# chensh236/ComputerVisionImageStich2

Measured on AMD Instinct MI355X. Metric: warp+blend MPix/s at 4096x4096x3 f32, higher is better.
Workload: dtype f32 (f64 accumulators)

## Files before the change

computervisionimagestich2_amd/capi.py:

```python
import ctypes as C
import os
import re

import numpy as np

_HERE = os.path.dirname(os.path.abspath(__file__))
LIB_PATH = os.environ.get("STITCH_LIB", os.path.join(_HERE, "libstitch_hip.so"))

KERNELS = ("compose", "seam", "mask", "vv_x_fwd", "vv_x_bwd", "vv_y_fwd", "vv_y_bwd", "decimate", "collapse_top", "collapse",
           "collapse_l0", "vv_xbyf", "vv_x_fwd_src", "coarse")
KERNEL_SYMBOLS = {"compose": "k_src_index (source-fused) / k_compose", "seam": "k_seam", "mask": "k_mask", "vv_x_fwd": "k_vv_x_fwd<T, false, false>", "vv_x_bwd": "k_vv_x_bwd",
                  "vv_y_fwd": "k_vv_y_fwd1 / k_vv_y_fwd", "vv_y_bwd": "k_vv_y_bwd_dec", "decimate": "k_decimate", "collapse_top": "k_blend_top",
                  "collapse": "k_collapse<float, false>", "collapse_l0": "k_collapse<T, true>", "vv_xbyf": "k_vv_xbyf<false, float, 0, false>", "vv_x_fwd_src": "k_vv_x_fwd<T, true, false>",
                  "coarse": "k_coarse"}


class StitchError(RuntimeError):
    def __init__(self, code, text):
        super().__init__(f"stitch error {code}: {text}")
        self.code = code


OK, ERR_ARG, ERR_EMPTY_MIDROW, ERR_ZERO_OVERLAP, ERR_PYRAMID, ERR_HIP, ERR_NO_DEVICE = 0, -1, -2, -3, -4, -5, -6
ERR_NO_MAP, ERR_CAPACITY = -7, -8
# ... 101 lines not shown
)

RIG_EXPOSURE_SIGNATURES = _signatures(
    ("stitch_rig_create_exposure", i32, vp, i32, i32, vp, i32, vp, vp, vp), ("stitch_rig_from_panorama_exposure", i32, vp, vp, i32, vp, vp, vp),
    ("stitch_dev_rig_stitch_exposure_u8", i32, vp, vp, i32, vp, vp, vp, vp, vp),
    ("stitch_dev_transfer_many_u8", i32, vp, vp, vp, i32, i32, i32, i32, i32, i32, i32, vp, vp, vp),
)

CALIBRATE_SIGNATURES = _signatures(
    ("stitch_calibrate_opts_default stitch_calibration_destroy", None, vp), ("stitch_dev_calibrate_u8", i32, vp, i32, i32, vp, vp, vp),
    ("stitch_dev_calibrate_from_features_u8", i32, vp, vp, i32, i32, vp, vp, vp), ("stitch_calibrate_u8", i32, vp, i32, i32, vp, vp),
    ("stitch_calibration_info", i32, vp, vp, vp, vp, vp, vp, vp), ("stitch_calibration_step_at", i32, vp, i32, vp),
    ("stitch_calibration_counts", i32, vp, vp, vp), ("stitch_calibration_step_support", i32, vp, i32, vp, vp),
    ("stitch_rig_from_calibration", i32, vp, vp, vp, vp),
)

RIG_SEAMS_SIGNATURES = _signatures(
    ("stitch_seam_from_sums", i32, i32, i32, i32, i32, i32, i32, vp), ("stitch_dev_pairs_seamed_*", i32, vp, vp, i32, vp, vp),
    ("stitch_rig_fix_seams stitch_rig_seams", i32, vp, vp, i32), ("stitch_rig_clear_seams", i32, vp),
    ("stitch_dev_rig_geometric_seams", i32, vp, vp, vp), ("stitch_dev_rig_coverage_u8", i32, vp, i32, i32, vp, vp),
    ("stitch_rig_step_canvas", i32, vp, i32, vp, vp),
)

_lib = None


def lib():
    global _lib
    if _lib is None:
        if not os.path.exists(LIB_PATH):
            raise ImportError(f"{LIB_PATH} is missing: build it with `python -c 'import __graft_entry__ as g; g.build()'` "
                              "(make -C computervisionimagestich2_amd/csrc). There is no CPU fallback.")
        try:
            import torch
        except ImportError:
            pass
        L = C.CDLL(LIB_PATH)
        for name, (res, args) in list(SIGNATURES.items()) + list(PANORAMA_SIGNATURES.items()) + list(RIG_SIGNATURES.items()) + list(EXPOSURE_SIGNATURES.items()) \
                + list(RIG_EXPOSURE_SIGNATURES.items()) + list(CALIBRATE_SIGNATURES.items()) + list(RIG_SEAMS_SIGNATURES.items()):
            try:
                f = getattr(L, name)
            except AttributeError:
                raise ImportError(f"{LIB_PATH} does not export {name}: it was built from another include/stitch.h") from None
            f.restype, f.argtypes = res, args
        L.stitch_plan_handoff_counts.restype, L.stitch_plan_handoff_counts.argtypes = i32, [vp, vp]
        if hasattr(L, "stitch_plan_g_flag_counts"):
            L.stitch_plan_g_flag_counts.restype, L.stitch_plan_g_flag_counts.argtypes = i32, [vp, vp]
        if hasattr(L, "stitch_plan_mask_row_counts"):
            L.stitch_plan_mask_row_counts.restype, L.stitch_plan_mask_row_counts.argtypes = i32, [vp, vp]
        if hasattr(L, "stitch_plan_index_counts"):
            L.stitch_plan_index_counts.restype, L.stitch_plan_index_counts.argtypes = i32, [vp, vp]
        _lib = L
    return _lib


def _chk(rc):
    if rc < 0:
        raise StitchError(rc, lib().stitch_last_error().decode())
    return rc


def _p(a):
    return a.ctypes.data_as(C.c_void_p)


def _fn(stem, a):
    sfx = {"uint8": "u8", "float32": "f32"}.get(str(a.dtype).rpartition(".")[2])
    if sfx is None:
        raise TypeError(f"unsupported pixel type {a.dtype}")
    return getattr(lib(), stem + sfx)


def _img(a):
    a = np.ascontiguousarray(a)
# ... 730 lines not shown
    _chk(lib().stitch_dev_finish_u8(_dp(result), result.shape[2], result.shape[1], num, den, _dp(hist), _stream()))
    return result


def dev_synth(w, h, frame_id, dtype, device=None):
    import torch
    out = torch.empty((3, h, w), dtype=dtype, device=device or torch.device("cuda", torch.cuda.current_device()))
    _chk(_fn("stitch_dev_synth_", out)(_dp(out), int(w), int(h), int(frame_id), _stream()))
    return out


def dev_check_fastdiv(w):
    t, m = C.c_ulonglong(), C.c_ulonglong()
    _chk(lib().stitch_dev_check_fastdiv(w, C.byref(t), C.byref(m)))
    return t.value, m.value


def dev_check_collapse_taps(w, h, probe):
    t, m = C.c_ulonglong(), C.c_ulonglong()
    _chk(lib().stitch_dev_check_collapse_taps(int(w), int(h), int(probe), C.byref(t), C.byref(m)))
    return t.value, m.value


def dev_quantize(src, out=None):
    import torch
    assert src.is_cuda and src.is_contiguous() and src.dtype == torch.float32
    out = torch.empty(src.shape, dtype=torch.uint8, device=src.device) if out is None else out
    _chk(lib().stitch_dev_quantize_u8(_dp(src), _dp(out), src.numel(), _stream()))
    return out


class _Handle:

    def close(self):
        if self._h:
            getattr(lib(), self._destroy)(self._h)
            self._h = C.c_void_p()

    def __del__(self):
        try:
            self.close()
        except Exception:
            pass


class Plan(_Handle):
# ... 96 lines not shown
    def clear_fault(self):
        _chk(lib().stitch_plan_clear_fault(self._h))

    def handoff_counts(self):
        out = (C.c_uint64 * 3)()
        _chk(lib().stitch_plan_handoff_counts(self._h, out))
        return tuple(int(v) for v in out)

    def g_flag_counts(self):
        out = (C.c_uint64 * 2)()
        _chk(lib().stitch_plan_g_flag_counts(self._h, out))
        return tuple(int(v) for v in out)

    def mask_row_counts(self):
        out = (C.c_uint64 * 2)()
        _chk(lib().stitch_plan_mask_row_counts(self._h, out))
        return tuple(int(v) for v in out)

    def index_counts(self):
        out = (C.c_uint32 * 3)()
        _chk(lib().stitch_plan_index_counts(self._h, out))
        return tuple(int(v) for v in out)

    def set_handoff_spin_limit(self, polls):
        _chk(lib().stitch_plan_set_handoff_spin_limit(self._h, int(polls)))

    def set_profiling_kernel(self, name):
        _chk(lib().stitch_plan_set_profiling_kernel(self._h, KERNELS.index(name)))

    def set_profiling(self, on):
        _chk(lib().stitch_plan_set_profiling(self._h, int(bool(on))))

    def read_profile(self):
        ms, n, l0 = (C.c_double * len(KERNELS))(), (C.c_int * len(KERNELS))(), (C.c_double * len(KERNELS))()
        _chk(lib().stitch_plan_read_profile(self._h, ms, n, l0))
        return {KERNELS[i]: (ms[i], n[i], l0[i]) for i in range(len(KERNELS))}


class Band(_Handle):
    _destroy = "stitch_band_destroy"

    def __init__(self, cw, ch, rank, nranks, split_levels, opts=None):
        self._h = C.c_void_p()
        _chk(lib().stitch_band_create(int(cw), int(ch), int(rank), int(nranks), int(split_levels), C.byref(_opts(opts)), C.byref(self._h)))
        self.cw, self.ch, self.rank, self.nranks, self.split_levels = int(cw), int(ch), int(rank), int(nranks), int(split_levels)
        tot = C.c_int()
# ... 346 lines not shown
```

computervisionimagestich2_amd/csrc/k_pyramid.inc:

```
__global__ __launch_bounds__(64) void k_deriche(float* __restrict__ data, float* __restrict__ Y, int N, size_t off,
                                                size_t line_stride, long lines_per_plane, size_t ps, long lines, DRK k) {
    const long line = (long)blockIdx.x * WAVE + threadIdx.x;
    if (line >= lines) return;
    const long plane = line / lines_per_plane, li = line % lines_per_plane;
    float* ptrX = data + plane * ps + li * line_stride;
    float* ptrY = Y + plane * ps + li * line_stride;
    float xp = *ptrX, yb, yp;
    yb = yp = (float)(k.coefp * xp);
    for (int m = 0; m < N; ++m) {
        const float xc = ptrX[(size_t)m * off];
        const float yc = k.a0 * xc + k.a1 * xp - k.b1 * yp - k.b2 * yb;
        ptrY[(size_t)m * off] = yc;
        xp = xc;
        yb = yp;
        yp = yc;
    }
    float xn, xa, yn, ya;
    xn = xa = ptrX[(size_t)(N - 1) * off];
    yn = ya = k.coefn * xn;
    for (int n = N - 1; n >= 0; --n) {
        const float xc = ptrX[(size_t)n * off];
        const float yc = k.a2 * xn + k.a3 * xa - k.b1 * yn - k.b2 * ya;
        xa = xn;
        xn = xc;
// ... 336 lines not shown
    template <typename PX>
    __device__ __forceinline__ NoShift4(const PX*, int, int, int, int, int, int) {}
    __device__ __forceinline__ void issue(int, float[4]) const {}
};
template <typename PX, bool ON>
struct Shift4If {
    typedef NoShift4 type;
};
template <typename PX>
struct Shift4If<PX, true> {
    typedef Shift4<PX> type;
};
template <typename PX, bool AD>
struct SrcRow4 {
    __amdgpu_buffer_rsrc_t fr;
    Shift4<PX> mo;
    typename Shift4If<PX, AD>::type fa;
    __device__ __forceinline__ SrcRow4(const PairArgs<PX>& pa, int pr, int c, int x0, int w)
        : mo(pa.mosaic[pr] + c * ((size_t)pa.mw[pr] * pa.mh[pr]), pa.mw[pr], pa.mh[pr], pa.ox[pr], pa.oy[pr], x0, w),
          fa(pa.frame[pr] + c * ((size_t)pa.fw[pr] * pa.fh[pr]), pa.fw[pr], pa.fh[pr], 0, 0, x0, w) {
        const size_t fe = (size_t)pa.fw[pr] * pa.fh[pr];
        fr = plane_rsrc(pa.frame[pr] + c * fe, fe);
    }
    __device__ __forceinline__ void issue(const u4 idx, int y, float a[4], float b[4]) const {
        if constexpr (AD)
            fa.issue(y, a);
        else {
#pragma unroll
            for (int j = 0; j < 4; ++j) a[j] = buf_raw<PX>(fr, idx[j]);
        }
#if STITCH_C4_ABLATE == 3 || STITCH_C4_ABLATE >= 8
        for (int j = 0; j < 4; ++j) b[j] = (float)y;
#else
        mo.issue(y, b);
#endif
    }
    __device__ __forceinline__ void finish(float a[4], float b[4]) const {
#pragma unroll
        for (int j = 0; j < 4; ++j) {
            a[j] = AD ? raw_to_px<PX>(a[j]) : warped_px<PX>(raw_to_px<PX>(a[j]));
            b[j] = raw_to_px<PX>(b[j]);
        }
    }
};
struct NoSrcRow4 {
    __device__ __forceinline__ NoSrcRow4(const NoPairArgs&, int, int, int, int) {}
    __device__ __forceinline__ void issue(const u4, int, float[4], float[4]) const {}
    __device__ __forceinline__ void finish(float[4], float[4]) const {}
};
template <typename OUT, bool DENSE, bool AD>
struct SrcRow4Of {
    typedef NoSrcRow4 type;
};
template <typename OUT, bool AD>
struct SrcRow4Of<OUT, true, AD> {
    typedef SrcRow4<OUT, AD> type;
};

#ifndef STITCH_C4_WAVES
#define STITCH_C4_WAVES 7
#endif
#ifndef STITCH_C4_PREFETCH
#define STITCH_C4_PREFETCH 0
#endif
#ifndef STITCH_C4_ABLATE
#define STITCH_C4_ABLATE 0
#endif
#ifndef STITCH_C4_OPAQUE_ALPHA
#define STITCH_C4_OPAQUE_ALPHA 1
#endif
typedef __attribute__((address_space(3))) f4 lds_f4;
template <typename OUT, bool DENSE, bool AD, bool GEN, bool MR = false>
__device__ __forceinline__ void collapse_cols4(const CollapseArgs<OUT, DENSE>& A, int c, int x0, int y0, int y1, int pr, float* sh, MaskRowsArg mr = MaskRowsArg{}) {
    const int pitch = A.pitch, sh_ = A.sh, spitch = A.spitch, opitch = A.opitch;
    const size_t ps = A.ps, sps = A.sps, ops = A.ops;
    const ExpandTab& tb = A.tb;
    const SeamDev* __restrict__ seam_l0 = A.seam_l0;
    const float* g = A.g_all + (size_t)collapse_slot(A, pr) * 7 * ps;
    const bool share = !DENSE && !seam_l0 && A.lockstep == 2;
    const float* sa = A.gn_all + ((size_t)pr * 7 + c) * sps;
    const float* sb = sa + 3 * sps;
    const float* se = A.en_all + ((size_t)pr * 3 + c) * sps;
    OUT* __restrict__ out = (DENSE ? A.outs.p[pr] : A.outs.p[0] + (size_t)pr * 3 * ops) + c * ops;
    uint8_t* __restrict__ out8 = DENSE && A.outs.q[pr] ? A.outs.q[pr] + c * ops : nullptr;
    const bool use_src = DENSE && A.use_src;
    const int s0 = tb.ix[x0];
    int o1 = 1, o2 = 1, o3 = 2;
    bool e1 = false, e2 = false, e3 = false;
    if constexpr (GEN) {
        const int4 ix4 = *reinterpret_cast<const int4*>(tb.ix + x0);
        o1 = ix4.y - ix4.x, o2 = ix4.z - ix4.x, o3 = ix4.w - ix4.x;
#ifndef STITCH_C4_NO_ENDTAP
        e1 = ix4.y >= A.sw - 1, e2 = ix4.z >= A.sw - 1, e3 = ix4.w >= A.sw - 1;
#endif
    }
#if STITCH_G_IGNORE_COARSER & 1
    const bool za = false, zb = false;
#else
    const bool za = g_span_flag(A.gzn, A.gncn, pr * 7 + c, s0, s0 + 3), zb = g_span_flag(A.gzn, A.gncn, pr * 7 + 3 + c, s0, s0 + 3);
#endif
#if STITCH_G_IGNORE_OWN & 1
    const bool zga = false, zgb = false;
#else
    const bool zga = !DENSE && g_span_flag(A.gz, A.gnc, pr * 7 + c, x0, x0), zgb = !DENSE && g_span_flag(A.gz, A.gnc, pr * 7 + 3 + c, x0, x0);
#endif
    const unsigned zsa = (unsigned)((size_t)A.zon - ((size_t)pr * 7 + c) * sps), zsb = (unsigned)((size_t)A.zon - ((size_t)pr * 7 + 3 + c) * sps);
    const size_t zg = (size_t)A.zo - (size_t)pr * 7 * ps;
    double axs[4];
    {
        const double2 a01 = *reinterpret_cast<const double2*>(tb.ax + x0), a23 = *reinterpret_cast<const double2*>(tb.ax + x0 + 2);
        axs[0] = a01.x, axs[1] = a01.y, axs[2] = a23.x, axs[3] = a23.y;
    }
    auto xrow = [&](int row, float X[3][4]) {
        const unsigned o = (unsigned)row * (unsigned)spitch + (unsigned)s0;
#if STITCH_C4_ABLATE == 1 || STITCH_C4_ABLATE >= 8
        const f4 v[3] = {f4{0.f, 0.f, 0.f, (float)o}, f4{0.f, 0.f, 0.f, 1.f}, f4{0.f, 0.f, 0.f, 2.f}};
#else
        const f4 v[3] = {*reinterpret_cast<const f4u*>(sa + (za ? zsa : o)), *reinterpret_cast<const f4u*>(sb + (zb ? zsb : o)), *reinterpret_cast<const f4u*>(se + o)};
#endif
#if STITCH_C4_OPAQUE_ALPHA
#pragma unroll
        for (int j = 0; j < 4; ++j) asm volatile("" : "+v"(axs[j]));
#endif
#pragma unroll
        for (int q = 0; q < 3; ++q) {
            if constexpr (GEN) {
                const float x_ = v[q].x, y_ = v[q].y, z_ = v[q].z, w_ = v[q].w;
                X[q][0] = lerp_ref(axs[0], x_, y_);
                const float a1 = o1 ? y_ : x_, a2 = o2 == 0 ? x_ : o2 == 1 ? y_ : z_, a3 = o3 == 0 ? x_ : o3 == 1 ? y_ : z_;
                X[q][1] = lerp_ref(axs[1], a1, e1 ? a1 : o1 ? z_ : y_);
                X[q][2] = lerp_ref(axs[2], a2, e2 ? a2 : o2 == 0 ? y_ : o2 == 1 ? z_ : w_);
                X[q][3] = lerp_ref(axs[3], a3, e3 ? a3 : o3 == 0 ? y_ : o3 == 1 ? z_ : w_);
            } else {
                X[q][0] = lerp_ref(axs[0], v[q].x, v[q].y);
                X[q][1] = lerp_ref(axs[1], v[q].y, v[q].z);
                X[q][2] = lerp_ref(axs[2], v[q].y, v[q].z);
                X[q][3] = lerp_ref(axs[3], v[q].z, v[q].w);
            }
        }
    };
    float X1[3][4], X2[3][4];
    int cur1 = -1, cur2 = -1;
    float m4[4] = {0.f, 0.f, 0.f, 0.f};
    if (seam_l0) {
        const SeamDev sd = seam_l0[pr];
#pragma unroll
        for (int j = 0; j < 4; ++j) m4[j] = mask_step(sd, x0 + j);
    }
    const typename SrcRow4Of<OUT, DENSE, AD>::type src(A.pa, pr, c, x0, A.w);
    bool mrow = false;
    auto row_issue = [&](int y, float ga[4], float gb[4], f4& vm) {
        const unsigned o = (unsigned)y * (unsigned)pitch + (unsigned)x0;
        if constexpr (MR)
            if (y == y0 || (y & 63) == 0) mrow = collapse_mask_row(mr, pr, x0, y);
        const unsigned om = MR && mrow ? (unsigned)x0 : o;
        if (use_src)
#if STITCH_C4_ABLATE == 2
            src.issue(u4{0u, 4u, 8u, 12u}, y, ga, gb);
#elif STITCH_C4_ABLATE >= 6
        {
            const unsigned e = ((unsigned)y * 4096u + (unsigned)(x0 - 2048)) * 4u;
            const u4 calc = x0 >= 2048 ? u4{e, e + 4u, e + 8u, e + 12u} : u4{0xfffffff0u, 0xfffffff0u, 0xfffffff0u, 0xfffffff0u};
            src.issue(c == 0 && STITCH_C4_ABLATE == 6 ? *reinterpret_cast<const u4*>(g + o) : STITCH_C4_ABLATE >= 8 ? u4{0u, 4u, 8u, 12u} : calc, y, ga, gb);
        }
#else
            src.issue(AD ? u4{0u, 0u, 0u, 0u} : *reinterpret_cast<const u4*>(g + o), y, ga, gb);
#endif
        else {
            const f4 va = *reinterpret_cast<const f4*>(g + (zga ? zg : o + c * ps)), vb = *reinterpret_cast<const f4*>(g + (zgb ? zg : o + (3 + c) * ps));
#pragma unroll
            for (int j = 0; j < 4; ++j) ga[j] = va[j], gb[j] = vb[j];
        }
        if (share) {
            if (c == 0) vm = *reinterpret_cast<const f4*>(g + om + 6 * ps);
        } else
#if STITCH_C4_ABLATE == 11
        if (!seam_l0) vm = c == 0 ? *reinterpret_cast<const f4*>(g + o + 6 * ps) : f4{0.5f, 0.5f, 0.5f, 0.5f};
#elif STITCH_C4_ABLATE == 12
        if (!seam_l0) vm = f4{0.5f, 0.5f, 0.5f, (float)y};
#else
        if (!seam_l0) vm = *reinterpret_cast<const f4*>(g + om + 6 * ps);
#endif
    };
    float ga[4], gb[4];
    f4 vm = {0.f, 0.f, 0.f, 0.f};
#if STITCH_C4_PREFETCH
    float gan[4], gbn[4];
    f4 vmn = {0.f, 0.f, 0.f, 0.f};
    row_issue(y0, gan, gbn, vmn);
#endif
    for (int y = y0; y < y1; ++y) {
        if (A.lockstep == 1) __builtin_amdgcn_s_barrier();
        const int iy = tb.iy[y], iy2 = iy < sh_ - 1 ? iy + 1 : iy;
        const double ay = tb.ay[y];
        if (iy != cur1) {
            if (iy == cur2) {
#pragma unroll
                for (int q = 0; q < 3; ++q)
#pragma unroll
                    for (int j = 0; j < 4; ++j) X1[q][j] = X2[q][j];
            } else
                xrow(iy, X1);
            cur1 = iy;
        }
        if (iy2 != cur2) {
            if (iy2 == cur1) {
#pragma unroll
                for (int q = 0; q < 3; ++q)
#pragma unroll
                    for (int j = 0; j < 4; ++j) X2[q][j] = X1[q][j];
            } else
                xrow(iy2, X2);
            cur2 = iy2;
        }
#if STITCH_C4_PREFETCH
#pragma unroll
        for (int j = 0; j < 4; ++j) ga[j] = gan[j], gb[j] = gbn[j];
        vm = vmn;
        if (y + 1 < y1) row_issue(y + 1, gan, gbn, vmn);
#else
        row_issue(y, ga, gb, vm);
#endif
        if (share) {
            lds_f4* slot = (lds_f4*)sh + (y & 1) * WAVE + (threadIdx.x & 63);
            if (c == 0) *slot = vm;
            asm volatile("s_waitcnt lgkmcnt(0)\n\ts_barrier" ::: "memory");
            vm = *slot;
        }
        if (use_src) src.finish(ga, gb);
        if (!seam_l0) {
#pragma unroll
            for (int j = 0; j < 4; ++j) m4[j] = vm[j];
        }
        float v4[4];
#pragma unroll
        for (int j = 0; j < 4; ++j) {
            const float ea = lerp_ref(ay, X1[0][j], X2[0][j]);
            const float eb = lerp_ref(ay, X1[1][j], X2[1][j]);
            const float ee = lerp_ref(ay, X1[2][j], X2[2][j]);
            const float la = ga[j] - ea;
            const float lb = gb[j] - eb;
            const float s_ = blend_ref(la, lb, m4[j]);
            float v = s_ + ee;
            if (v > 255.f)
                v = 255.f;
            else if (v < 0.f)
                v = 0.f;
            v4[j] = v;
        }
#if STITCH_C4_ABLATE == 4
        if (!(v4[0] != v4[0] || v4[3] != v4[3])) continue;
#endif
        if constexpr (DENSE)
        {
#if STITCH_C4_ABLATE == 5
            *reinterpret_cast<f4u*>(&out[(size_t)y * opitch + x0]) = f4u{v4[0], v4[1], v4[2], v4[3]};
            continue;
#endif
            store4<OUT>(&out[(size_t)y * opitch + x0], v4, A.u8_words != 0);
            if (sizeof(OUT) == 4 && out8) store4<uint8_t>(&out8[(size_t)y * opitch + x0], v4, A.u8_words != 0);
        }
        else
            *reinterpret_cast<f4*>(&out[(size_t)y * opitch + x0]) = f4{v4[0], v4[1], v4[2], v4[3]};
    }
}

constexpr int C4_SUB = 8, C4_THREADS = 3 * WAVE;
__host__ __device__ inline int c4_padded_blocks(int nb4, int swizzle) { return swizzle && nb4 >= 8 ? (nb4 + 7) & ~7 : nb4; }
template <typename OUT, bool DENSE, bool AD = false, bool GEN = false, bool MR = false>
__global__ __launch_bounds__(C4_THREADS, STITCH_C4_WAVES) void k_collapse4(CollapseArgs<OUT, DENSE> A, int nb4, int ncb, MaskRowsArg mr = MaskRowsArg{}) {
    const int pr = blockIdx.z;
    __shared__ __attribute__((aligned(16))) float c4_sh[2 * WAVE * 4];
    const int nb4p = c4_padded_blocks(nb4, A.swizzle);
    if ((int)blockIdx.x < nb4p) {
        const int c = __builtin_amdgcn_readfirstlane(threadIdx.x >> 6);
        int blk = blockIdx.x, strip = blockIdx.y;
        const int nb8 = nb4p & ~7;
        const int S8 = (int)gridDim.y & ~7;
        if (A.swizzle >= 2 && blk < nb8 && (int)blockIdx.y < S8) {
            const unsigned first = gridDim.x * (blockIdx.y + gridDim.y * blockIdx.z);
            const int xcd = (int)((first + (unsigned)blk) & 7u), t = (int)blockIdx.y * (nb8 >> 3) + (blk >> 3);
            strip = xcd * (S8 >> 3) + t / nb8;
            blk = t % nb8;
        } else if (A.swizzle && blk < nb8) {
            const unsigned first = gridDim.x * (blockIdx.y + gridDim.y * blockIdx.z);
            const int xcd = (int)((first + (unsigned)blk) & 7u), k = blk >> 3, K = nb8 >> 3, s0 = (int)blockIdx.y & ~7;
            if (s0 + 8 <= (int)gridDim.y) {
                strip = s0 + xcd;
                blk = ((int)blockIdx.y - s0) * K + k;
            } else
                blk = xcd * K + k;
        }
        const int y0 = strip * A.crows, y1 = min(y0 + A.crows, A.h);
        const int x0 = A.xa + (blk * WAVE + (threadIdx.x & 63)) * 4;
        if (blk < nb4 && x0 < A.xb) collapse_cols4<OUT, DENSE, AD, GEN, MR>(A, c, x0, y0, y1, pr, c4_sh, mr);
    } else {
        const int y0 = blockIdx.y * A.crows, y1 = min(y0 + A.crows, A.h);
        const int r = blockIdx.x - nb4p, cb = r % ncb, sub = r / ncb, rows = (A.crows + C4_SUB - 1) / C4_SUB;
        int x = cb * C4_THREADS + threadIdx.x;
        if (x >= A.xa) x += A.xb - A.xa;
        const int ya = y0 + sub * rows, yb = min(ya + rows, y1);
#if STITCH_C4_ABLATE == 9 || STITCH_C4_ABLATE == 10
        if (A.h < 0)
#endif
        if (x < (DENSE ? A.w : A.pitch) && ya < yb) collapse_cols1<OUT, DENSE, MR>(A, x, ya, yb, pr, mr);
    }
}

template <bool MR = false>
__global__ __launch_bounds__(256) void k_collapse_px(CollapseArgs<float, false> A, MaskRowsArg mr = MaskRowsArg{}) {
    const int x = blockIdx.x * blockDim.x + threadIdx.x, y = blockIdx.y, pr = blockIdx.z;
    if (x >= A.pitch) return;
    const float* g = A.g_all + (size_t)pr * 7 * A.ps;
    const float* gn = A.gn_all + (size_t)pr * 7 * A.sps;
    const float* en = A.en_all + (size_t)pr * 3 * A.sps;
    float* e = A.outs.p[0] + (size_t)pr * 3 * A.ops;
    const size_t i = (size_t)y * A.pitch + x;
    if (x >= A.w) {
// ... 47 lines not shown
```

computervisionimagestich2_amd/csrc/stitch_call_form.h:

```cpp
#pragma once
#include <stddef.h>
#include <stdint.h>

#include <algorithm>
#include <cstdlib>
#include <cstring>
#include <vector>

#include "stitch.h"

#ifndef STITCH_CROWS
#define STITCH_CROWS 8
#endif

namespace sk {

constexpr int TS = 64;
constexpr int YCH = 8, YCOLS = 2 * TS;
constexpr int XY_MAXNC = 1024;
constexpr int CROWS = STITCH_CROWS;
constexpr int CO_MAXL = 16;
constexpr int CO_MAXSIDE = 512;
constexpr int CO_TABN = 192;
constexpr int MAXB = 16;
// ... 67 lines not shown
        bool reg = b < nblk && sw >= 2 && sh >= 2;
        for (int x0 = b * 256; reg && x0 < (b + 1) * 256; x0 += 4) {
            const int s_ = idx[x0];
            reg = idx[x0 + 1] == s_ + 1 && idx[x0 + 2] == s_ + 1 && idx[x0 + 3] == s_ + 2 && s_ + 3 <= sw - 1;
        }
        if (reg && run_a < 0) run_a = b;
        if (!reg && run_a >= 0) {
            if (b - run_a > best_b - best_a) best_a = run_a, best_b = b;
            run_a = -1;
        }
    }
    if (best_b > best_a) *xa = best_a * 256, *xb = best_b * 256;
}

inline void general_range(const std::vector<int32_t>& idx, int w, int sw, int sh, int* xb) {
    *xb = 0;
    if (sw < 4 || sh < 2) return;
    int x0 = 0;
    for (; x0 + 3 < w; x0 += 4) {
        const int s_ = idx[x0];
        if (!(idx[x0 + 1] >= s_ && idx[x0 + 2] >= idx[x0 + 1] && idx[x0 + 3] >= idx[x0 + 2] && idx[x0 + 3] - s_ <= 2 && s_ >= 0 && s_ + 1 <= sw - 1)) break;
    }
    *xb = x0 / 256 * 256;
}

inline int pyramid_sizes(int w, int h, int level_rule, int* lw, int* lh) {
    if (w <= 0 || h <= 0) return 0;
    const int len = level_rule ? (w < h ? w : h) : (w >= h ? w : h);
    int levels = 0;
    while ((len >> (levels + 1)) > 0) ++levels;
    if (levels < 1 || levels > 32) return -1;
    int cw = w, ch = h;
    for (int i = 0; i < levels; ++i) {
        if (cw <= 0 || ch <= 0) return -(2 + i);
        if (lw) lw[i] = cw;
        if (lh) lh[i] = ch;
        cw /= 2;
        ch /= 2;
    }
    return levels;
}

struct PlanShape {
    int cw = 0, ch = 0, L = 0;
    int cap = 1;
    stitch_blend_opts opts{};
// ... 486 lines not shown
```

computervisionimagestich2_amd/csrc/stitch_hip.hip:

```cpp
#include <hip/hip_runtime.h>

#include <cmath>
#include <cstdarg>
#include <cstdio>
#include <cstdlib>
#include <algorithm>
#include <cstring>
#include <atomic>
#include <condition_variable>
#include <functional>
#include <list>
#include <mutex>
#include <string>
#include <thread>
#include <vector>

#include "stitch.h"
#include "stitch_g_flags.h"
#include "stitch_index_plane.h"
#include "stitch_handoff.h"
#include "stitch_mask_rows.h"
#include "stitch_panorama.h"
#include "stitch_rig.h"
#include "stitch_exposure.h"
#include "stitch_rig_exposure.h"
#include "stitch_calibrate.h"
#include "stitch_rig_seams.h"
#include "stitch_kernels.hpp"

#pragma clang fp contract(off)

using namespace sk;

namespace {

thread_local std::string g_err;


int fail(int code, const char* fmt, ...) {
    char buf[512];
    va_list ap;
    va_start(ap, fmt);
// ... 122 lines not shown
    uint8_t* zt = nullptr;
    uint8_t* gz[2] = {nullptr, nullptr};
    uint8_t* mr[2] = {nullptr, nullptr};
    const float* zero_page = nullptr;
    int wf_max_wgs = WF_MAX_WGS;
    unsigned wf_spin_limit = WF_SPIN_LIMIT;
    int wf_early_read = 1;
    double* ckpt = nullptr;
    unsigned long long* d7_dbg = nullptr;
    int d7_dbg_chunks = 0;
    unsigned long long* xy_dbg = nullptr;
    int xy_dbg_nc = 0;
    unsigned long long* wf_dbg = nullptr;
    unsigned* h_wf_abort = nullptr;
    unsigned wf_abort_seen = 0;
    float* side = nullptr;
    unsigned long long* co_dbg = nullptr;
    SeamDev* d_seam = nullptr;
    SeamDev* h_seam = nullptr;
    IndexKey* idx_keys = nullptr;
    unsigned* idx_head = nullptr;
    unsigned* h_idx_head = nullptr;
    bool last_idx = false;
    hipStream_t last_stream = nullptr;
    bool pending = false;
    VVK vvk{};
    DRK drk{};
    bool profiling = false;
    int prof_only = -1;
    std::vector<ProfRec> recs;
    std::vector<hipEvent_t> free_events;
};

Tuning sk::Tuning::from_env() {
    Tuning t{};
    t.wavefront = env_int("STITCH_WAVEFRONT");
    t.no_fuse = env_int("STITCH_NO_FUSE") > 0;
    t.no_src_fuse = env_int("STITCH_NO_SRC_FUSE") > 0;
    t.no_zero_tiles = env_int("STITCH_NO_ZERO_TILES") > 0;
    t.crows_l0 = env_int("STITCH_CROWS_L0");
    t.crows_ln = env_int("STITCH_CROWS_LN");
    t.collapse4 = env_int("STITCH_COLLAPSE4");
    t.xbyf_wgs = env_int("STITCH_XBYF_WGS");
    t.xbyf_spin_limit = env_int("STITCH_XBYF_SPIN_LIMIT");
    t.xbyf_early = env_int("STITCH_XBYF_EARLY");
    t.y2 = env_int("STITCH_Y2") > 0;
// ... 317 lines not shown
    const int L = p->L, n = c.n;
    if (!c.coarse) {
        const Level& t = p->lv[L - 1];
        StageTimer tm(p, s, STITCH_K_COLLAPSE_TOP, L - 1);
        k_blend_top<<<grid_xy(t.pitch, t.h, n), 256, 0, s>>>(t.g, t.pitch, t.h, t.ps, t.e);
        if (L == 1) k_emit_top<OUT><<<grid_xy(t.w, t.h, n), 256, 0, s>>>(t.e, t.w, t.h, t.pitch, t.ps, outs);
    }
    for (int l = c.l_end - 1; l >= 0; --l) {
        const LevelForm& f = c.lv[l];
        const Level& a = p->lv[l];
        const Level& nx = p->lv[l + 1];
        StageTimer tm(p, s, l == 0 ? STITCH_K_COLLAPSE_L0 : STITCH_K_COLLAPSE, l);
        const ZeroTiles none{};
        const ZeroTiles gz = f.g_in ? g_cols(p->gz[l - 1], a.w) : none, gzn = f.g_out ? g_cols(p->gz[l], nx.w) : none;
        const ZeroTiles mrz = f.c_mr ? mask_rows(p->mr[l - 1], a.w, a.h) : none;
        const int cols = l == 0 ? a.w : a.pitch, strips = (a.h + f.crows - 1) / f.crows;
        const MaskRowsArg mra{mrz.flags, mrz.NC, mrz.NR};
        if (l == 0) {
            CollapseArgs<OUT, true> A{a.g, a.w, a.h, a.pitch, a.ps, nx.g, nx.e, nx.w, nx.h, nx.pitch, nx.ps, {a.ix, a.ax, a.iy, a.ay}, outs,
                                      a.w, (size_t)a.w * a.h, p->planes_in ? nullptr : p->d_seam, pa, c.src ? 1 : 0, f.crows, f.xa, f.xb, 1,
                                      c.c4_lock, c.c4_swizzle};
            A.gzn = gzn.flags, A.gncn = gzn.NC, A.zon = (unsigned)(7 * (size_t)p->cap * nx.ps);
            launch_collapse(A, CollapseKind{c.src && c.a_dense, f.gen, false, false, false}, cols, strips, n, mra, s);
        } else {
            OutPtrs<float> eo{};
            eo.p[0] = a.e;
            CollapseArgs<float, false> A{a.g, a.w, a.h, a.pitch, a.ps, nx.g, nx.e, nx.w, nx.h, nx.pitch, nx.ps, {a.ix, a.ax, a.iy, a.ay}, eo,
                                         a.pitch, a.ps, nullptr, NoPairArgs{}, 0, f.crows, f.xa, f.xb, 1, c.c4_lock, c.c4_swizzle};
            A.gz = gz.flags, A.gnc = gz.NC, A.zo = (unsigned)(7 * (size_t)p->cap * a.ps);
            A.gzn = gzn.flags, A.gncn = gzn.NC, A.zon = (unsigned)(7 * (size_t)p->cap * nx.ps);
            launch_collapse(A, CollapseKind{false, f.gen, f.px, f.c_mr, false}, cols, strips, n, mra, s);
        }
    }
    return launch_check("collapse");
}

template <typename PX>
int run_seam_mask(stitch_plan* p, int n, hipStream_t s, const PairArgs<PX>& pa, bool src, const SeamInts* given) {
    const Level& a = p->lv[0];
    if (given) {
        StageTimer t(p, s, STITCH_K_SEAM, 0);
        k_seam_given<<<1, 64, 0, s>>>(*given, n, a.w, p->opts.seam_rule, p->d_seam);
    } else {
        StageTimer t(p, s, STITCH_K_SEAM, 0);
        k_seam<PX><<<n, n == 1 ? 1024 : 256, 0, s>>>(a.g, a.w, a.h, a.pitch, a.ps, p->opts.seam_rule, p->d_seam, pa, src ? 1 : 0);
    }
// ... 1160 lines not shown
int stitch_plan_g_flag_counts(stitch_plan* p, uint64_t out[2]) {
    if (!p || !out) return fail(STITCH_ERR_ARG, "null plan or output");
    if (p->pending) {
        HIPCHK(hipStreamSynchronize(p->last_stream));
        p->pending = false;
    }
    for (int i = 0; i < 2; ++i) {
        out[i] = 0;
        if (!p->last_form.lv[i].g_out || !p->gz[i] || p->last_n <= 0) continue;
        std::vector<uint8_t> h((size_t)7 * p->last_n * ((p->lv[i + 1].w + TS - 1) / TS));
        HIPCHK(hipMemcpy(h.data(), p->gz[i], h.size(), hipMemcpyDeviceToHost));
        for (uint8_t f : h) out[i] += f != 0;
    }
    return STITCH_OK;
}

int stitch_plan_index_counts(stitch_plan* p, uint32_t out[3]) {
    if (!p || !out) return fail(STITCH_ERR_ARG, "null plan or output");
    if (p->pending) {
        HIPCHK(hipStreamSynchronize(p->last_stream));
        p->pending = false;
    }
    for (int i = 0; i < 3; ++i) out[i] = p->last_idx ? p->h_idx_head[i] : 0u;
    return STITCH_OK;
}

int stitch_plan_mask_row_counts(stitch_plan* p, uint64_t out[2]) {
    if (!p || !out) return fail(STITCH_ERR_ARG, "null plan or output");
    if (p->pending) {
        HIPCHK(hipStreamSynchronize(p->last_stream));
        p->pending = false;
    }
    for (int i = 0; i < 2; ++i) {
        out[i] = 0;
        if (!p->last_form.lv[i].mr_out || !p->mr[i] || p->last_n <= 0) continue;
        const ZeroTiles m = mask_rows(p->mr[i], p->lv[i + 1].w, p->lv[i + 1].h);
        std::vector<uint8_t> h((size_t)p->last_n * m.NC * m.NR);
        HIPCHK(hipMemcpy(h.data(), p->mr[i], h.size(), hipMemcpyDeviceToHost));
        for (uint8_t f : h) out[i] += f != 0;
    }
    return STITCH_OK;
}

int stitch_plan_clear_fault(stitch_plan* p) {
    if (!p) return fail(STITCH_ERR_ARG, "null plan");
    if (p->pending) {
// ... 449 lines not shown
            CollapseArgs<float, false> A{(const float*)(base + off[0]), w, h, pitch, ps, (const float*)(base + off[1]), (const float*)(base + off[2]), sw, sh, spitch, sps,
                                         tb, eo, pitch, ps, nullptr, NoPairArgs{}, 0, crows, 0, v == 0 ? gxb : 0, 1, 0, 1};
            launch_collapse(A, CollapseKind{false, true, false, false, false}, pitch, strips, 1, MaskRowsArg{}, nullptr);
        }
        ok = hipDeviceSynchronize() == hipSuccess && hipMemcpy(o1.data(), base + off[3], bytes[3], hipMemcpyDeviceToHost) == hipSuccess &&
             hipMemcpy(o2.data(), base + off[4], bytes[4], hipMemcpyDeviceToHost) == hipSuccess;
    }
    const hipError_t e = ok ? hipSuccess : hipGetLastError();
    (void)hipFree(base);
    if (!ok) return fail(STITCH_ERR_HIP, "check_collapse_taps: %s", hipGetErrorString(e));
    unsigned long long n = 0, bad = 0;
    for (size_t q = 0; q < 3; ++q)
        for (int y = 0; y < h; ++y)
            for (int x = 0; x < w; ++x, ++n) {
                uint32_t a, b;
                std::memcpy(&a, &o1[q * ps + (size_t)y * pitch + x], 4);
                std::memcpy(&b, &o2[q * ps + (size_t)y * pitch + x], 4);
                bad += a != b;
            }
    *compared = n;
    *mismatches = bad;
    return STITCH_OK;
}
int stitch_dev_quantize_u8(const float* d_src, uint8_t* d_dst, size_t n, void* stream) {
    int rc = need_device();
    if (rc) return rc;
    if (!d_src || !d_dst || n == 0) return fail(STITCH_ERR_ARG, "quantize: bad argument");
    k_quantize<<<eq_grid((n + 3) / 4), 256, 0, as_stream(stream)>>>(d_src, d_dst, n);
    return launch_check("k_quantize");
}

}

#include "stitch_band.inc"
#include "stitch_match.inc"
#include "stitch_ransac.inc"
#include "stitch_sift.inc"
#include "stitch_chain.inc"
#include "stitch_panorama.inc"
#include "stitch_rig.inc"
#include "stitch_exposure.inc"
#include "stitch_rig_exposure.inc"
#include "stitch_calibrate.inc"
#include "stitch_rig_seams.inc"
```

Measured before the change: 26570.

## Specialize level-0 collapse blocks lying wholly on one side of the seam

When a 256-column block of the level-0 collapse sits entirely on one side of the seam step, a templated SIDE variant of collapse_cols4 loads and expands only the selected image's Laplacian and coarse rows. The other image's source, Laplacian and coarse-level reads are skipped, along with its interpolation work. Where a signed-zero corner case could make the blend differ bit for bit, a wave-level redo path recomputes the full two-sided blend. This adds three template instantiations, which grows code size and register pressure, plus diagnostic APIs that count sides and check bit equality.

```diff
diff --git a/computervisionimagestich2_amd/capi.py b/computervisionimagestich2_amd/capi.py
--- a/computervisionimagestich2_amd/capi.py
+++ b/computervisionimagestich2_amd/capi.py
@@ -147,6 +147,10 @@
     ("stitch_rig_step_canvas", i32, vp, i32, vp, vp),
 )
 
+COLLAPSE_SIDES_SIGNATURES = _signatures(
+    ("stitch_plan_collapse_sides", i32, vp, i32, vp), ("stitch_dev_check_collapse_sides", i32, i32, i32, i32, i32, i32, vp, vp, vp),
+)
+
 _lib = None
 
 
@@ -175,6 +179,10 @@
             L.stitch_plan_mask_row_counts.restype, L.stitch_plan_mask_row_counts.argtypes = i32, [vp, vp]
         if hasattr(L, "stitch_plan_index_counts"):
             L.stitch_plan_index_counts.restype, L.stitch_plan_index_counts.argtypes = i32, [vp, vp]
+        for name, (res, args) in COLLAPSE_SIDES_SIGNATURES.items():
+            if hasattr(L, name):
+                f = getattr(L, name)
+                f.restype, f.argtypes = res, args
         _lib = L
     return _lib
 
@@ -951,6 +959,12 @@
     return t.value, m.value
 
 
+def dev_check_collapse_sides(w, h, probe, branch, seam_x):
+    t, m, n = C.c_ulonglong(), C.c_ulonglong(), (C.c_int * 3)()
+    _chk(lib().stitch_dev_check_collapse_sides(int(w), int(h), int(probe), int(branch), int(seam_x), C.byref(t), C.byref(m), n))
+    return t.value, m.value, tuple(int(v) for v in n)
+
+
 def dev_quantize(src, out=None):
     import torch
     assert src.is_cuda and src.is_contiguous() and src.dtype == torch.float32
@@ -1093,6 +1107,11 @@
         _chk(lib().stitch_plan_index_counts(self._h, out))
         return tuple(int(v) for v in out)
 
+    def collapse_sides(self, pair=0):
+        out = (C.c_int * 3)()
+        _chk(lib().stitch_plan_collapse_sides(self._h, int(pair), out))
+        return tuple(int(v) for v in out)
+
     def set_handoff_spin_limit(self, polls):
         _chk(lib().stitch_plan_set_handoff_spin_limit(self._h, int(polls)))
 
diff --git a/computervisionimagestich2_amd/csrc/k_pyramid.inc b/computervisionimagestich2_amd/csrc/k_pyramid.inc
--- a/computervisionimagestich2_amd/csrc/k_pyramid.inc
+++ b/computervisionimagestich2_amd/csrc/k_pyramid.inc
@@ -382,18 +382,23 @@
         const size_t fe = (size_t)pa.fw[pr] * pa.fh[pr];
         fr = plane_rsrc(pa.frame[pr] + c * fe, fe);
     }
+    template <int SIDE = 0>
     __device__ __forceinline__ void issue(const u4 idx, int y, float a[4], float b[4]) const {
-        if constexpr (AD)
-            fa.issue(y, a);
-        else {
-#pragma unroll
-            for (int j = 0; j < 4; ++j) a[j] = buf_raw<PX>(fr, idx[j]);
-        }
+        if constexpr (SIDE != 2) {
+            if constexpr (AD)
+                fa.issue(y, a);
+            else {
+#pragma unroll
+                for (int j = 0; j < 4; ++j) a[j] = buf_raw<PX>(fr, idx[j]);
+            }
+        }
+        if constexpr (SIDE != 1) {
 #if STITCH_C4_ABLATE == 3 || STITCH_C4_ABLATE >= 8
-        for (int j = 0; j < 4; ++j) b[j] = (float)y;
-#else
-        mo.issue(y, b);
-#endif
+            for (int j = 0; j < 4; ++j) b[j] = (float)y;
+#else
+            mo.issue(y, b);
+#endif
+        }
     }
     __device__ __forceinline__ void finish(float a[4], float b[4]) const {
 #pragma unroll
@@ -405,6 +410,7 @@
 };
 struct NoSrcRow4 {
     __device__ __forceinline__ NoSrcRow4(const NoPairArgs&, int, int, int, int) {}
+    template <int SIDE = 0>
     __device__ __forceinline__ void issue(const u4, int, float[4], float[4]) const {}
     __device__ __forceinline__ void finish(float[4], float[4]) const {}
 };
@@ -430,7 +436,7 @@
 #define STITCH_C4_OPAQUE_ALPHA 1
 #endif
 typedef __attribute__((address_space(3))) f4 lds_f4;
-template <typename OUT, bool DENSE, bool AD, bool GEN, bool MR = false>
+template <typename OUT, bool DENSE, bool AD, bool GEN, bool MR = false, int SIDE = 0>
 __device__ __forceinline__ void collapse_cols4(const CollapseArgs<OUT, DENSE>& A, int c, int x0, int y0, int y1, int pr, float* sh, MaskRowsArg mr = MaskRowsArg{}) {
     const int pitch = A.pitch, sh_ = A.sh, spitch = A.spitch, opitch = A.opitch;
     const size_t ps = A.ps, sps = A.sps, ops = A.ops;
@@ -457,7 +463,7 @@
 #if STITCH_G_IGNORE_COARSER & 1
     const bool za = false, zb = false;
 #else
-    const bool za = g_span_flag(A.gzn, A.gncn, pr * 7 + c, s0, s0 + 3), zb = g_span_flag(A.gzn, A.gncn, pr * 7 + 3 + c, s0, s0 + 3);
+    const bool za = SIDE != 2 && g_span_flag(A.gzn, A.gncn, pr * 7 + c, s0, s0 + 3), zb = SIDE != 1 && g_span_flag(A.gzn, A.gncn, pr * 7 + 3 + c, s0, s0 + 3);
 #endif
 #if STITCH_G_IGNORE_OWN & 1
     const bool zga = false, zgb = false;
@@ -471,12 +477,28 @@
         const double2 a01 = *reinterpret_cast<const double2*>(tb.ax + x0), a23 = *reinterpret_cast<const double2*>(tb.ax + x0 + 2);
         axs[0] = a01.x, axs[1] = a01.y, axs[2] = a23.x, axs[3] = a23.y;
     }
+    auto xl4 = [&](const f4 v, float X[4]) {
+        if constexpr (GEN) {
+            const float x_ = v.x, y_ = v.y, z_ = v.z, w_ = v.w;
+            X[0] = lerp_ref(axs[0], x_, y_);
+            const float a1 = o1 ? y_ : x_, a2 = o2 == 0 ? x_ : o2 == 1 ? y_ : z_, a3 = o3 == 0 ? x_ : o3 == 1 ? y_ : z_;
+            X[1] = lerp_ref(axs[1], a1, e1 ? a1 : o1 ? z_ : y_);
+            X[2] = lerp_ref(axs[2], a2, e2 ? a2 : o2 == 0 ? y_ : o2 == 1 ? z_ : w_);
+            X[3] = lerp_ref(axs[3], a3, e3 ? a3 : o3 == 0 ? y_ : o3 == 1 ? z_ : w_);
+        } else {
+            X[0] = lerp_ref(axs[0], v.x, v.y);
+            X[1] = lerp_ref(axs[1], v.y, v.z);
+            X[2] = lerp_ref(axs[2], v.y, v.z);
+            X[3] = lerp_ref(axs[3], v.z, v.w);
+        }
+    };
     auto xrow = [&](int row, float X[3][4]) {
         const unsigned o = (unsigned)row * (unsigned)spitch + (unsigned)s0;
 #if STITCH_C4_ABLATE == 1 || STITCH_C4_ABLATE >= 8
         const f4 v[3] = {f4{0.f, 0.f, 0.f, (float)o}, f4{0.f, 0.f, 0.f, 1.f}, f4{0.f, 0.f, 0.f, 2.f}};
 #else
-        const f4 v[3] = {*reinterpret_cast<const f4u*>(sa + (za ? zsa : o)), *reinterpret_cast<const f4u*>(sb + (zb ? zsb : o)), *reinterpret_cast<const f4u*>(se + o)};
+        const f4 v[3] = {SIDE != 2 ? *reinterpret_cast<const f4u*>(sa + (za ? zsa : o)) : f4{0.f, 0.f, 0.f, 0.f},
+                         SIDE != 1 ? *reinterpret_cast<const f4u*>(sb + (zb ? zsb : o)) : f4{0.f, 0.f, 0.f, 0.f}, *reinterpret_cast<const f4u*>(se + o)};
 #endif
 #if STITCH_C4_OPAQUE_ALPHA
 #pragma unroll
@@ -484,19 +506,16 @@
 #endif
 #pragma unroll
         for (int q = 0; q < 3; ++q) {
-            if constexpr (GEN) {
-                const float x_ = v[q].x, y_ = v[q].y, z_ = v[q].z, w_ = v[q].w;
-                X[q][0] = lerp_ref(axs[0], x_, y_);
-                const float a1 = o1 ? y_ : x_, a2 = o2 == 0 ? x_ : o2 == 1 ? y_ : z_, a3 = o3 == 0 ? x_ : o3 == 1 ? y_ : z_;
-                X[q][1] = lerp_ref(axs[1], a1, e1 ? a1 : o1 ? z_ : y_);
-                X[q][2] = lerp_ref(axs[2], a2, e2 ? a2 : o2 == 0 ? y_ : o2 == 1 ? z_ : w_);
-                X[q][3] = lerp_ref(axs[3], a3, e3 ? a3 : o3 == 0 ? y_ : o3 == 1 ? z_ : w_);
-            } else {
-                X[q][0] = lerp_ref(axs[0], v[q].x, v[q].y);
-                X[q][1] = lerp_ref(axs[1], v[q].y, v[q].z);
-                X[q][2] = lerp_ref(axs[2], v[q].y, v[q].z);
-                X[q][3] = lerp_ref(axs[3], v[q].z, v[q].w);
-            }
+            if ((q == 0 && SIDE == 2) || (q == 1 && SIDE == 1)) continue;
+            xl4(v[q], X[q]);
+        }
+    };
+    auto xcopy = [&](float D[3][4], const float S[3][4]) {
+#pragma unroll
+        for (int q = 0; q < 3; ++q) {
+            if ((q == 0 && SIDE == 2) || (q == 1 && SIDE == 1)) continue;
+#pragma unroll
+            for (int j = 0; j < 4; ++j) D[q][j] = S[q][j];
         }
     };
     float X1[3][4], X2[3][4];
@@ -524,12 +543,23 @@
             src.issue(c == 0 && STITCH_C4_ABLATE == 6 ? *reinterpret_cast<const u4*>(g + o) : STITCH_C4_ABLATE >= 8 ? u4{0u, 4u, 8u, 12u} : calc, y, ga, gb);
         }
 #else
-            src.issue(AD ? u4{0u, 0u, 0u, 0u} : *reinterpret_cast<const u4*>(g + o), y, ga, gb);
+        {
+            u4 idx = {0u, 0u, 0u, 0u};
+            if constexpr (!AD && SIDE != 2) idx = *reinterpret_cast<const u4*>(g + o);
+            src.template issue<SIDE>(idx, y, ga, gb);
+        }
 #endif
         else {
-            const f4 va = *reinterpret_cast<const f4*>(g + (zga ? zg : o + c * ps)), vb = *reinterpret_cast<const f4*>(g + (zgb ? zg : o + (3 + c) * ps));
-#pragma unroll
-            for (int j = 0; j < 4; ++j) ga[j] = va[j], gb[j] = vb[j];
+            if constexpr (SIDE != 2) {
+                const f4 va = *reinterpret_cast<const f4*>(g + (zga ? zg : o + c * ps));
+#pragma unroll
+                for (int j = 0; j < 4; ++j) ga[j] = va[j];
+            }
+            if constexpr (SIDE != 1) {
+                const f4 vb = *reinterpret_cast<const f4*>(g + (zgb ? zg : o + (3 + c) * ps));
+#pragma unroll
+                for (int j = 0; j < 4; ++j) gb[j] = vb[j];
+            }
         }
         if (share) {
             if (c == 0) vm = *reinterpret_cast<const f4*>(g + om + 6 * ps);
@@ -542,7 +572,7 @@
         if (!seam_l0) vm = *reinterpret_cast<const f4*>(g + om + 6 * ps);
 #endif
     };
-    float ga[4], gb[4];
+    float ga[4] = {0.f, 0.f, 0.f, 0.f}, gb[4] = {0.f, 0.f, 0.f, 0.f};
     f4 vm = {0.f, 0.f, 0.f, 0.f};
 #if STITCH_C4_PREFETCH
     float gan[4], gbn[4];
@@ -554,22 +584,16 @@
         const int iy = tb.iy[y], iy2 = iy < sh_ - 1 ? iy + 1 : iy;
         const double ay = tb.ay[y];
         if (iy != cur1) {
-            if (iy == cur2) {
-#pragma unroll
-                for (int q = 0; q < 3; ++q)
-#pragma unroll
-                    for (int j = 0; j < 4; ++j) X1[q][j] = X2[q][j];
-            } else
+            if (iy == cur2)
+                xcopy(X1, X2);
+            else
                 xrow(iy, X1);
             cur1 = iy;
         }
         if (iy2 != cur2) {
-            if (iy2 == cur1) {
-#pragma unroll
-                for (int q = 0; q < 3; ++q)
-#pragma unroll
-                    for (int j = 0; j < 4; ++j) X2[q][j] = X1[q][j];
-            } else
+            if (iy2 == cur1)
+                xcopy(X2, X1);
+            else
                 xrow(iy2, X2);
             cur2 = iy2;
         }
@@ -593,20 +617,90 @@
             for (int j = 0; j < 4; ++j) m4[j] = vm[j];
         }
         float v4[4];
-#pragma unroll
-        for (int j = 0; j < 4; ++j) {
-            const float ea = lerp_ref(ay, X1[0][j], X2[0][j]);
-            const float eb = lerp_ref(ay, X1[1][j], X2[1][j]);
-            const float ee = lerp_ref(ay, X1[2][j], X2[2][j]);
-            const float la = ga[j] - ea;
-            const float lb = gb[j] - eb;
-            const float s_ = blend_ref(la, lb, m4[j]);
-            float v = s_ + ee;
-            if (v > 255.f)
-                v = 255.f;
-            else if (v < 0.f)
-                v = 0.f;
-            v4[j] = v;
+        if constexpr (SIDE == 0) {
+#pragma unroll
+            for (int j = 0; j < 4; ++j) {
+                const float ea = lerp_ref(ay, X1[0][j], X2[0][j]);
+                const float eb = lerp_ref(ay, X1[1][j], X2[1][j]);
+                const float ee = lerp_ref(ay, X1[2][j], X2[2][j]);
+                const float la = ga[j] - ea;
+                const float lb = gb[j] - eb;
+                const float s_ = blend_ref(la, lb, m4[j]);
+                float v = s_ + ee;
+                if (v > 255.f)
+                    v = 255.f;
+                else if (v < 0.f)
+                    v = 0.f;
+                v4[j] = v;
+            }
+        } else {
+            constexpr int K = SIDE == 1 ? 0 : 1;
+            const float* gk = SIDE == 1 ? ga : gb;
+            bool redo = false;
+#pragma unroll
+            for (int j = 0; j < 4; ++j) {
+                const float ek = lerp_ref(ay, X1[K][j], X2[K][j]);
+                const float ee = lerp_ref(ay, X1[2][j], X2[2][j]);
+                const float lk = gk[j] - ek;
+                float v = lk + ee;
+                redo = redo || ((__float_as_uint(lk) << 1) == 0u && __float_as_uint(ee) == 0x80000000u);
+                if (v > 255.f)
+                    v = 255.f;
+                else if (v < 0.f)
+                    v = 0.f;
+                v4[j] = v;
+            }
+#ifndef STITCH_C4_NO_SIDE_REDO
+            if (__builtin_expect(__any(redo), 0)) {
+                int xr = x0;
+                asm volatile("" : "+v"(xr));
+                constexpr int D = 1 - K;
+                const float* sd_ = D == 0 ? sa : sb;
+                const unsigned zsd = D == 0 ? zsa : zsb;
+#if STITCH_G_IGNORE_COARSER & 1
+                const bool zd = false;
+#else
+                const bool zd = g_span_flag(A.gzn, A.gncn, pr * 7 + 3 * D + c, tb.ix[xr], tb.ix[xr] + 3);
+#endif
+                float gd[4] = {0.f, 0.f, 0.f, 0.f}, gu[4] = {0.f, 0.f, 0.f, 0.f};
+                const unsigned o = (unsigned)y * (unsigned)pitch + (unsigned)xr;
+                if (use_src) {
+                    const typename SrcRow4Of<OUT, DENSE, AD>::type srd(A.pa, pr, c, xr, A.w);
+                    u4 idx = {0u, 0u, 0u, 0u};
+                    if constexpr (!AD && D == 0) idx = *reinterpret_cast<const u4*>(g + o);
+                    if constexpr (D == 0) {
+                        srd.template issue<1>(idx, y, gd, gu);
+                        srd.finish(gd, gu);
+                    } else {
+                        srd.template issue<2>(idx, y, gu, gd);
+                        srd.finish(gu, gd);
+                    }
+                } else {
+                    const f4 vd = *reinterpret_cast<const f4*>(g + o + (3 * D + c) * ps);
+#pragma unroll
+                    for (int j = 0; j < 4; ++j) gd[j] = vd[j];
+                }
+                float D1[4], D2[4];
+                const unsigned sr = (unsigned)tb.ix[xr];
+                xl4(*reinterpret_cast<const f4u*>(sd_ + (zd ? zsd : (unsigned)iy * (unsigned)spitch + sr)), D1);
+                xl4(*reinterpret_cast<const f4u*>(sd_ + (zd ? zsd : (unsigned)iy2 * (unsigned)spitch + sr)), D2);
+#pragma unroll
+                for (int j = 0; j < 4; ++j) {
+                    const float ek = lerp_ref(ay, X1[K][j], X2[K][j]);
+                    const float ed = lerp_ref(ay, D1[j], D2[j]);
+                    const float ee = lerp_ref(ay, X1[2][j], X2[2][j]);
+                    const float lk = gk[j] - ek;
+                    const float ld = gd[j] - ed;
+                    const float s_ = SIDE == 1 ? blend_ref(lk, ld, m4[j]) : blend_ref(ld, lk, m4[j]);
+                    float v = s_ + ee;
+                    if (v > 255.f)
+                        v = 255.f;
+                    else if (v < 0.f)
+                        v = 0.f;
+                    v4[j] = v;
+                }
+            }
+#endif
         }
 #if STITCH_C4_ABLATE == 4
         if (!(v4[0] != v4[0] || v4[3] != v4[3])) continue;
@@ -653,7 +747,30 @@
         }
         const int y0 = strip * A.crows, y1 = min(y0 + A.crows, A.h);
         const int x0 = A.xa + (blk * WAVE + (threadIdx.x & 63)) * 4;
-        if (blk < nb4 && x0 < A.xb) collapse_cols4<OUT, DENSE, AD, GEN, MR>(A, c, x0, y0, y1, pr, c4_sh, mr);
+        if (blk < nb4 && x0 < A.xb) {
+            int side = 0;
+#ifndef STITCH_NO_C4_SIDES
+            if constexpr (DENSE) {
+                if (A.seam_l0) {
+                    const SeamDev& sd = A.seam_l0[pr];
+                    const int xf = A.xa + blk * (4 * WAVE);
+                    side = __builtin_amdgcn_readfirstlane(c4_block_side(sd.branch, sd.start, sd.thr, xf, min(xf + 4 * WAVE - 1, A.xb - 1)));
+#ifdef STITCH_C4_WRONG_SIDE
+                    side = side ? 3 - side : 0;
+#endif
+                }
+            }
+#endif
+            if constexpr (DENSE) {
+                if (side == 1)
+                    collapse_cols4<OUT, DENSE, AD, GEN, MR, 1>(A, c, x0, y0, y1, pr, c4_sh, mr);
+                else if (side == 2)
+                    collapse_cols4<OUT, DENSE, AD, GEN, MR, 2>(A, c, x0, y0, y1, pr, c4_sh, mr);
+                else
+                    collapse_cols4<OUT, DENSE, AD, GEN, MR, 0>(A, c, x0, y0, y1, pr, c4_sh, mr);
+            } else
+                collapse_cols4<OUT, DENSE, AD, GEN, MR>(A, c, x0, y0, y1, pr, c4_sh, mr);
+        }
     } else {
         const int y0 = blockIdx.y * A.crows, y1 = min(y0 + A.crows, A.h);
         const int r = blockIdx.x - nb4p, cb = r % ncb, sub = r / ncb, rows = (A.crows + C4_SUB - 1) / C4_SUB;
diff --git a/computervisionimagestich2_amd/csrc/stitch_call_form.h b/computervisionimagestich2_amd/csrc/stitch_call_form.h
--- a/computervisionimagestich2_amd/csrc/stitch_call_form.h
+++ b/computervisionimagestich2_amd/csrc/stitch_call_form.h
@@ -113,6 +113,18 @@
         if (!(idx[x0 + 1] >= s_ && idx[x0 + 2] >= idx[x0 + 1] && idx[x0 + 3] >= idx[x0 + 2] && idx[x0 + 3] - s_ <= 2 && s_ >= 0 && s_ + 1 <= sw - 1)) break;
     }
     *xb = x0 / 256 * 256;
+}
+
+constexpr int c4_step_at(int branch, int start, double thr, int x) { return branch == 0 ? ((double)x < thr ? 1 : 0) : (x >= start ? 1 : 0); }
+constexpr int c4_block_side(int branch, int start, double thr, int xf, int xl) {
+    return c4_step_at(branch, start, thr, xf) != c4_step_at(branch, start, thr, xl) ? 0 : c4_step_at(branch, start, thr, xf) ? 1 : 2;
+}
+inline void c4_side_counts(int branch, int start, double thr, int xa, int xb, int sides, int counts[3]) {
+    counts[0] = counts[1] = counts[2] = 0;
+    for (int xf = xa; xf < xb; xf += 256) {
+        const int side = sides ? c4_block_side(branch, start, thr, xf, std::min(xf + 255, xb - 1)) : 0;
+        ++counts[side == 1 ? 0 : side == 2 ? 1 : 2];
+    }
 }
 
 inline int pyramid_sizes(int w, int h, int level_rule, int* lw, int* lh) {
diff --git a/computervisionimagestich2_amd/csrc/stitch_hip.hip b/computervisionimagestich2_amd/csrc/stitch_hip.hip
--- a/computervisionimagestich2_amd/csrc/stitch_hip.hip
+++ b/computervisionimagestich2_amd/csrc/stitch_hip.hip
@@ -18,6 +18,7 @@
 #include "stitch.h"
 #include "stitch_g_flags.h"
 #include "stitch_index_plane.h"
+#include "stitch_collapse_sides.h"
 #include "stitch_handoff.h"
 #include "stitch_mask_rows.h"
 #include "stitch_panorama.h"
@@ -186,6 +187,8 @@
     unsigned* idx_head = nullptr;
     unsigned* h_idx_head = nullptr;
     bool last_idx = false;
+    int c4_l0_xa = 0, c4_l0_xb = 0;
+    bool c4_l0_sides = false;
     hipStream_t last_stream = nullptr;
     bool pending = false;
     VVK vvk{};
@@ -549,6 +552,12 @@
                                       c.c4_lock, c.c4_swizzle};
             A.gzn = gzn.flags, A.gncn = gzn.NC, A.zon = (unsigned)(7 * (size_t)p->cap * nx.ps);
             launch_collapse(A, CollapseKind{c.src && c.a_dense, f.gen, false, false, false}, cols, strips, n, mra, s);
+            p->c4_l0_xa = A.xa, p->c4_l0_xb = A.xb;
+#ifdef STITCH_NO_C4_SIDES
+            p->c4_l0_sides = false;
+#else
+            p->c4_l0_sides = A.seam_l0 != nullptr;
+#endif
         } else {
             OutPtrs<float> eo{};
             eo.p[0] = a.e;
@@ -1755,6 +1764,19 @@
         p->pending = false;
     }
     for (int i = 0; i < 3; ++i) out[i] = p->last_idx ? p->h_idx_head[i] : 0u;
+    return STITCH_OK;
+}
+
+int stitch_plan_collapse_sides(stitch_plan* p, int pair, int counts[3]) {
+    if (!p || !counts) return fail(STITCH_ERR_ARG, "null plan or output");
+    if (pair < 0 || pair >= std::max(1, p->last_n))
+        return fail(STITCH_ERR_ARG, "collapse_sides: pair %d outside the %d pair(s) of the plan's last call", pair, p->last_n);
+    if (p->pending) {
+        HIPCHK(hipStreamSynchronize(p->last_stream));
+        p->pending = false;
+    }
+    const SeamDev& sd = p->h_seam[pair];
+    c4_side_counts(sd.branch, sd.start, sd.thr, p->c4_l0_xa, p->last_n > 0 ? p->c4_l0_xb : p->c4_l0_xa, p->c4_l0_sides ? 1 : 0, counts);
     return STITCH_OK;
 }
 
@@ -2250,6 +2272,88 @@
     *mismatches = bad;
     return STITCH_OK;
 }
+int stitch_dev_check_collapse_sides(int w, int h, int probe, int branch, int seam_x, unsigned long long* compared, unsigned long long* mismatches,
+                                    int counts[3]) {
+    int rc = need_device();
+    if (rc) return rc;
+    if (w < 256 || (w & 1) || h < 4 || (h & 1) || w > 16384 || h > 16384 || probe < 0 || probe > 1 || branch < 0 || branch > 1 || seam_x < 0 || seam_x > w ||
+        !compared || !mismatches)
+        return fail(STITCH_ERR_ARG, "check_collapse_sides: even w >= 256, even h >= 4 (both <= 16384), probe 0 or 1, branch 0 or 1, 0 <= seam_x <= w");
+    const int sw = w / 2, sh = h / 2, pitch = round_up(w, 64), spitch = round_up(sw, 64);
+    const size_t ps = (size_t)pitch * h, sps = (size_t)spitch * sh, ops = (size_t)w * h;
+    std::vector<int32_t> ix, iy;
+    std::vector<double> ax, ay;
+    expand_table(sw, w, ix, ax);
+    expand_table(sh, h, iy, ay);
+    int gxb = 0;
+    general_range(ix, w, sw, sh, &gxb);
+    if (gxb < 256) return fail(STITCH_ERR_ARG, "check_collapse_sides: no block of this width takes the four-column path");
+    std::vector<float> g(7 * ps + (size_t)pitch * 64, 0.f), gn(7 * sps + (size_t)spitch * 64, 0.f), en(3 * sps + (size_t)spitch * 64, 0.f);
+    uint32_t lcg = 0x51DE5u ^ (uint32_t)(w * 31 + h);
+    auto rnd = [&]() {
+        lcg = lcg * 1664525u + 1013904223u;
+        return ((int)(lcg >> 8) % 60001 - 30000) / 117.0f;
+    };
+    for (size_t q = 0; q < 6; ++q)
+        for (int y = 0; y < h; ++y)
+            for (int x = 0; x < w; ++x)
+                g[q * ps + (size_t)y * pitch + x] = !probe ? rnd() : ((q < 3 ? (x + y + (int)q) % 3 : (x / 3 + y + (int)q) % 2) == 0 ? -0.0f : 0.0f);
+    if (!probe)
+        for (size_t q = 0; q < 6; ++q)
+            for (int y = 0; y < sh; ++y)
+                for (int x = 0; x < sw; ++x) gn[q * sps + (size_t)y * spitch + x] = rnd();
+    for (size_t q = 0; q < 3; ++q)
+        for (int y = 0; y < sh; ++y)
+            for (int x = 0; x < sw; ++x) {
+                const int k = (x + y + (int)q) % 3;
+                en[q * sps + (size_t)y * spitch + x] = !probe ? rnd() : k == 0 ? -0.0f : k == 1 ? -1.401298464e-45f : 0.0f;
+            }
+    SeamDev sd{};
+    sd.branch = branch, sd.start = seam_x, sd.thr = (double)seam_x;
+    const size_t bytes[] = {g.size() * 4, gn.size() * 4, en.size() * 4, 3 * ops * 4, 3 * ops * 4, (size_t)w * 4, (size_t)w * 8, (size_t)h * 4, (size_t)h * 8, sizeof sd};
+    size_t off[11] = {0};
+    for (int i = 0; i < 10; ++i) off[i + 1] = off[i] + align256(bytes[i]);
+    char* base = nullptr;
+    HIPCHK(hipMalloc((void**)&base, off[10] + 256));
+    auto up = [&](int i, const void* src) { return hipMemcpy(base + off[i], src, bytes[i], hipMemcpyHostToDevice) == hipSuccess; };
+    bool ok = up(0, g.data()) && up(1, gn.data()) && up(2, en.data()) && up(5, ix.data()) && up(6, ax.data()) && up(7, iy.data()) && up(8, ay.data()) && up(9, &sd) &&
+              hipMemset(base + off[3], 0xff, 2 * align256(bytes[3])) == hipSuccess;
+    std::vector<float> o1(3 * ops), o2(3 * ops);
+    int got[3] = {0, 0, 0};
+    if (ok) {
+        const ExpandTab tb{(const int32_t*)(base + off[5]), (const double*)(base + off[6]), (const int32_t*)(base + off[7]), (const double*)(base + off[8])};
+        const int crows = 8, strips = (h + crows - 1) / crows;
+        for (int v = 0; v < 2; ++v) {
+            OutPtrs<float> eo{};
+            eo.p[0] = (float*)(base + off[3 + v]);
+            CollapseArgs<float, true> A{(const float*)(base + off[0]), w, h, pitch, ps, (const float*)(base + off[1]), (const float*)(base + off[2]), sw, sh, spitch, sps,
+                                        tb, eo, w, ops, (const SeamDev*)(base + off[9]), PairArgs<float>{}, 0, crows, 0, v == 0 ? gxb : 0, 1, 0, 1};
+            launch_collapse(A, CollapseKind{false, true, false, false, false}, w, strips, 1, MaskRowsArg{}, nullptr);
+            if (v == 0) {
+#ifdef STITCH_NO_C4_SIDES
+                c4_side_counts(sd.branch, sd.start, sd.thr, A.xa, A.xb, 0, got);
+#else
+                c4_side_counts(sd.branch, sd.start, sd.thr, A.xa, A.xb, 1, got);
+#endif
+            }
+        }
+        ok = hipDeviceSynchronize() == hipSuccess && hipMemcpy(o1.data(), base + off[3], bytes[3], hipMemcpyDeviceToHost) == hipSuccess &&
+             hipMemcpy(o2.data(), base + off[4], bytes[4], hipMemcpyDeviceToHost) == hipSuccess;
+    }
+    const hipError_t e = ok ? hipSuccess : hipGetLastError();
+    (void)hipFree(base);
+    if (!ok) return fail(STITCH_ERR_HIP, "check_collapse_sides: %s", hipGetErrorString(e));
+    *compared = (unsigned long long)o1.size();
+    *mismatches = 0;
+    for (size_t i = 0; i < o1.size(); ++i) {
+        uint32_t a, b;
+        std::memcpy(&a, &o1[i], 4);
+        std::memcpy(&b, &o2[i], 4);
+        *mismatches += a != b;
+    }
+    if (counts) counts[0] = got[0], counts[1] = got[1], counts[2] = got[2];
+    return STITCH_OK;
+}
 int stitch_dev_quantize_u8(const float* d_src, uint8_t* d_dst, size_t n, void* stream) {
     int rc = need_device();
     if (rc) return rc;
diff --git a/include/stitch_collapse_sides.h b/include/stitch_collapse_sides.h
--- /dev/null
+++ b/include/stitch_collapse_sides.h
@@ -0,0 +1,17 @@
+#ifndef STITCH_COLLAPSE_SIDES_H
+#define STITCH_COLLAPSE_SIDES_H
+#include <stdint.h>
+
+#include "stitch.h"
+
+#ifdef __cplusplus
+extern "C" {
+#endif
+int stitch_plan_collapse_sides(stitch_plan *plan, int pair, int counts[3]);
+
+int stitch_dev_check_collapse_sides(int w, int h, int probe, int branch, int seam_x, unsigned long long *compared, unsigned long long *mismatches,
+                                    int counts[3]);
+#ifdef __cplusplus
+}
+#endif
+#endif
```

New measurement: 27520 (median of 6 runs). 3.6% higher.
